# vribeiro1/artspeech

Measured on AMD Instinct MI355X. Metric: articulator-frames/sec (fwd+bwd), higher is better.
Workload: dtype f32

## Files before the change

artspeech_amd/_lib.py:

```python
import ctypes as C
import os

import torch

_HERE = os.path.dirname(os.path.abspath(__file__))
LIB_PATH = os.path.join(_HERE, "libartspeech_hip.so")

c_f32p = C.c_void_p


class Dims(C.Structure):
    _fields_ = [("vocab", C.c_int32), ("n_art", C.c_int32), ("embed", C.c_int32), ("hidden", C.c_int32),
                ("n_samp", C.c_int32), ("simple", C.c_int32)]


class Layout(C.Structure):
    _fields_ = [("embedding", C.c_int64),
                ("w_ih", C.c_int64 * 2), ("b_ih", C.c_int64 * 2), ("w_hh", C.c_int64 * 2), ("b_hh", C.c_int64 * 2),
                ("lin_w", C.c_int64), ("lin_b", C.c_int64),
                ("ln1_g", C.c_int64), ("ln1_b", C.c_int64), ("w1", C.c_int64), ("b1", C.c_int64),
                ("ln2_g", C.c_int64), ("ln2_b", C.c_int64), ("w2", C.c_int64), ("b2", C.c_int64),
                ("ln3_g", C.c_int64), ("ln3_b", C.c_int64), ("w3", C.c_int64), ("b3", C.c_int64),
                ("total", C.c_int64)]

# ... 22 lines not shown

class MultiMlp(C.Structure):
    _fields_ = [("groups", C.c_int32), ("rows", C.c_int32), ("layers", C.c_int32), ("h1", C.c_int32), ("h2", C.c_int32),
                ("k_max", C.c_int32), ("n_max", C.c_int32), ("latent", C.c_int32),
                ("dims", C.c_void_p), ("params", C.c_void_p), ("in_mode", C.c_int32), ("in_scale", C.c_float),
                ("x", C.c_void_p), ("x_r", C.c_int64), ("x_g", C.c_int64), ("in_idx", C.c_void_p),
                ("out_mode", C.c_int32), ("act", C.c_int32), ("y", C.c_void_p), ("y_r", C.c_int64), ("y_g", C.c_int64),
                ("out_idx", C.c_void_p), ("own_ptr", C.c_void_p), ("own", C.c_void_p), ("win", C.c_void_p),
                ("ws", C.c_void_p), ("ws_floats", C.c_int64), ("dy", C.c_void_p), ("dx", C.c_void_p), ("dparams", C.c_void_p)]


class Pca(C.Structure):
    _fields_ = [("groups", C.c_int32), ("features", C.c_int32), ("k_max", C.c_int32), ("batch", C.c_int32),
                ("k", C.c_void_p), ("x", C.c_void_p), ("rows", C.c_int64), ("x_r", C.c_int64), ("x_g", C.c_int64),
                ("order", C.c_void_p), ("n_seen", C.c_int64), ("state", C.c_void_p),
                ("components", C.c_void_p), ("singular_values", C.c_void_p), ("explained_variance", C.c_void_p),
                ("explained_variance_ratio", C.c_void_p), ("noise_variance", C.c_void_p),
                ("ws", C.c_void_p), ("ws_floats", C.c_int64)]


class Stream(C.c_void_p):
    from_param = C.c_void_p.from_param


_P, _S, _I32, _I64, _F, _D = C.c_void_p, Stream, C.c_int32, C.c_int64, C.c_float, C.c_double
_DIMS, _LAY = C.POINTER(Dims), C.POINTER(Layout)

PROTOTYPES = {
    "as_version": (C.c_char_p, []),
    "as_arch": (C.c_char_p, []),
    "as_last_error": (C.c_char_p, []),
    "as_artspeech_layout": (_I32, [_DIMS, _LAY]),
    "as_artspeech_workspace_floats": (_I64, [_DIMS, _I32, _I32]),
    "as_artspeech_fwd": (_I32, [_DIMS, _P, _P, _I64, _P, _I32, _I32, _P, _P, _I32, C.POINTER(Opts), _S]),
    "as_artspeech_bwd": (_I32, [_DIMS, _P, _P, _I64, _P, _I32, _I32, _P, _P, _P, _P, C.POINTER(Opts), _S]),
    "as_artspeech_dw2": (_I32, [_DIMS, _P, _I32, _I32, _P, _P, _S]),
    "as_gru_bidir_fwd": (_I32, [_P, _P, _I64, _P, _P, _P, _I32, _I32, _I32, _P, _P, _S]),
    "as_gru_bidir_bwd": (_I32, [_P, _P, _P, _P, _P, _I32, _I32, _I32, _P, _P, _S]),
    "as_gemm_f32": (_I32, [C.POINTER(Gemm), _S]),
    "as_linear_planes_floats": (_I64, [_I32, _I32]),
    "as_linear_fwd": (_I32, [_P, _I64, _P, _I64, _P, _P, _I64, _I32, _I32, _I32, _I32, _P, _S]),
    "as_layernorm_fwd_blockres": (_I32, [_P, _P, _P, _P, _I32, _I64, _I32, _I32, _S]),
    "as_head_workspace_floats": (_I64, [_DIMS, _I64]),
    "as_head_fwd": (_I32, [_DIMS, _LAY, _P, _P, _I64, _P, _P, _I32, _S]),
    "as_head_bwd": (_I32, [_DIMS, _LAY, _P, _P, _P, _I64, _P, _P, _P, _S]),
    "as_euclid_fwd": (_I32, [_P, _P, _I64, _I32, _I32, _P, _S]),
    "as_euclid_bwd": (_I32, [_P, _P, _P, _I64, _I32, _I32, _P, _S]),
    "as_euclid_masked_partials": (_I32, []),
    "as_euclid_masked_fwd_bwd": (_I32, [_P, _P, _I64, _P, _I32, _I32, _I32, _I32, _F, _P, _P, _P, _S]),
    "as_euclid_masked_fwd_bwd_presigmoid": (_I32, [_P, _P, _I64, _P, _I32, _I32, _I32, _I32, _F, _P, _P, _P, _S]),
    "as_p2cp_fwd": (_I32, [_P, _I64, _I64, _I64, _I32, _P, _I64, _I64, _I64, _I32, _I64, _P, _S]),
    "as_p2cp_bwd": (_I32, [_P, _I64, _I64, _I64, _I32, _P, _I64, _I64, _I64, _I32, _I64, _P, _P, _I64, _I64, _I64, _P, _I64, _I64, _I64,
                           _S]),
    "as_p2cp_masked_partials": (_I32, []),
    "as_p2cp_masked_fwd_bwd": (_I32, [_P, _P, _I64, _P, _I32, _I32, _I32, _I32, _F, _P, _P, _P, _S]),
    "as_p2cp_utterance_mean": (_I32, [_P, _P, _I32, _I32, _I32, _F, _P, _S]),
    "as_pearson_fwd": (_I32, [_P, _I64, _I64, _P, _I64, _I64, _I32, _I32, _I32, _I32, _F, _P, _P, _S]),
    "as_tract_variables_fwd": (_I32, [_P, _I64, _I32, _I32, _P, _I32, _P, _P, _P, _P, _S]),
    "as_area_function_fwd": (_I32, [_P, _P, _I64, _I64, _I64, _I64, _I32, _D, _D, _P, _P, _S]),
    "as_evenly_spaced_fx": (_I32, [_P, _P, _I64, _I32, _I32, _P, _S]),
    "as_adam_step": (_I32, [_P, _P, _P, _P, _I64, _F, _F, _F, _F, _F, _I64, _F, _S]),
    "as_dropout_fwd": (_I32, [_P, _P, _I64, _F, C.c_uint64, _S]),
    "as_layernorm_fwd": (_I32, [_P, _P, _P, _P, _P, _P, _P, _I64, _I32, _I64, _S]),
    "as_fold_ln": (_I32, [_P, _P, _P, _P, _P, _P, _I32, _I32, _I32, _S]),
    "as_attn_softmax": (_I32, [_P, _I64, _I32, _I32, _I32, _I32, _F, _P, _P, _S]),
    "as_embed_posenc": (_I32, [_P, _I64, _P, _P, _P, _I64, _I32, _I32, _S]),
    "as_attn_softmax_bwd": (_I32, [_P, _P, _I64, _I32, _I32, _F, _S]),
    "as_attention_supported": (_I32, [_I32, _I32, _I32, _I32]),
    "as_attention_fwd": (_I32, [_P, _P, _P, _P, _P, _P, _P, _P, _I32, _I32, _I32, _I32, _I32, _I32, _F, _S]),
    "as_attention_fwd_causal": (_I32, [_P, _P, _P, _P, _P, _P, _P, _P, _I32, _I32, _I32, _I32, _I32, _I32, _F, _S]),
    "as_attention_bwd_ds": (_I32, [_P, _P, _P, _P, _P, _I32, _I32, _I32, _I32, _I32, _I32, _F, _S]),
    "as_attention_bwd_ds_causal": (_I32, [_P, _P, _P, _P, _P, _I32, _I32, _I32, _I32, _I32, _I32, _F, _S]),
    "as_attn_softmax_bwd_t": (_I32, [_P, _P, _P, _P, _P, _I32, _I32, _I32, _I32, _I32, _I32, _F, _S]),
    "as_group_reduce": (_I32, [_P, _P, _I32, _I32, _I64, _P, _S]),
    "as_layernorm_bwd": (_I32, [_P, _P, _P, _P, _P, _I64, _I32, _S]),
    "as_unfold_ln": (_I32, [_P, _P, _P, _P, _P, _P, _P, _P, _I32, _I32, _I32, _S]),
    "as_relu_bwd": (_I32, [_P, _P, _P, _I64, _S]),
    "as_add": (_I32, [_P, _P, _P, _I64, _S]),
    "as_row_scale": (_I32, [_P, _P, _P, _I64, _I32, _S]),
    "as_copy_f32": (_I32, [_P, _P, _I64, _S]),
    "as_set_overlap": (None, [_I32]),
    "as_set_matrix_arith": (None, [_I32]),
    "as_get_matrix_arith": (_I32, []),
    "as_conv3x3_stem": (_I32, [_P, _I64, _I64, _I64, _I64, _P, _P, _P, _P, _I32, _I32, _I32, _I32, _S]),
    "as_conv3x3_c32": (_I32, [_P, _P, _P, _P, _P, _I32, _I32, _I32, _S]),
    "as_ln_feat_gelu": (_I32, [_P, _P, _P, _P, _I64, _I32, _I32, _S]),
    "as_gelu": (_I32, [_P, _P, _I64, _S]),
    "as_lstm_bidir_fwd": (_I32, [_P, _P, _I64, _P, _P, _P, _I32, _I32, _I32, _P, _P, _S]),
    "as_lstm_bidir_bwd": (_I32, [_P, _P, _P, _P, _I32, _I32, _I32, _P, _S]),
    "as_gru_unidir_fwd": (_I32, [_P, _P, _P, _P, _I32, _I32, _I32, _P, _S]),
    "as_gru_unidir_fwd_gates": (_I32, [_P, _P, _P, _P, _I32, _I32, _I32, _P, _P, _S]),
    "as_gru_unidir_bwd": (_I32, [_P, _P, _P, _P, _P, _I32, _I32, _I32, _P, _P, _S]),
    "as_ln_feat_gelu_bwd": (_I32, [_P, _P, _P, _P, _P, _P, _I64, _I32, _I32, _S]),
    "as_conv3x3_stem_bwd": (_I32, [_P, _P, _P, _I64, _I64, _I64, _I64, _I32, _I32, _I32, _I32, _S]),
    "as_gelu_bwd": (_I32, [_P, _P, _P, _P, _I64, _I32, _S]),
    "as_conv3x3_c32_wgrad": (_I32, [_P, _P, _P, _P, _I32, _I32, _I32, _P, _I64, _S]),
    "as_conv3x3_stem_wgrad": (_I32, [_P, _I64, _I64, _I64, _I64, _P, _P, _P, _I32, _I32, _I32, _I32, _P, _I64, _S]),
    "as_ln_feat_gelu_param_grad": (_I32, [_P, _P, _P, _P, _I64, _I32, _I32, _P, _P, _P, _I64, _S]),
    "as_layernorm_param_grad": (_I32, [_P, _P, _I64, _I32, _P, _P, _P, _I64, _S]),
    "as_ctc_workspace_floats": (_I64, [_I32, _I32, _I32]),
    "as_ctc_loss": (_I32, [_P, _I64, _I64, _I32, _I32, _I32, _I32, _P, _I64, _P, _P, _I32, _I32, _I32, _P, _I64, _P, _S]),
    "as_ctc_grad": (_I32, [_P, _I64, _I64, _I32, _I32, _I32, _I32, _P, _I64, _P, _P, _I32, _I32, _P, _I64, _P, _P, _I32, _P, _I64,
                           _I64, _S]),
    "as_decode_top1": (_I32, [_P, _I64, _I64, _I32, _I32, _I32, _P, _I32, _P, _P, _P, _S]),
    "as_edit_distance": (_I32, [_P, _I32, _P, _P, _I32, _P, _I32, _P, _I32, _P, _S]),
    "as_align_workspace_bytes": (_I64, [_I32, _I32, _I32]),
    "as_align_counts": (_I32, [_P, _I32, _P, _P, _I32, _P, _I32, _P, _I32, _I32, _P, _P, _P, _I64, _S]),
    "as_confusion_counts": (_I32, [_P, _I32, _P, _I32, _P, _I32, _P, _I32, _I32, _P, _S]),
    "as_intersect_semipolar_grid":(_I32, [_P, _P, _I64, _I32, _I32, _I32, _P, _P, _P, _S]),
    "as_artspeech_wait_head_grads": (_I32, [_P, _P]),
    "as_gather_pad_rows": (_I32, [_P, _P, _P, _I32, _I32, _I64, _I32, _D, _P, _S]),
    "as_lin_debug_stamps": (None, [_P, _I64]),
    "as_gru_debug_stamps": (None, [_P]),
    "as_multi_mlp_supported": (_I32, [_I32, _I32, _I32, _I32, _I32]),
    "as_multi_mlp_param_floats": (_I64, [_I32, _I32, _I32, _I32, _I32]),
    "as_multi_mlp_workspace_floats": (_I64, [C.POINTER(MultiMlp), _I32]),
    "as_multi_mlp_fwd": (_I32, [C.POINTER(MultiMlp), _S]),
    "as_multi_mlp_bwd": (_I32, [C.POINTER(MultiMlp), _S]),
    "as_pca_supported": (_I32, [_I32, _I32]),
    "as_pca_workspace_floats": (_I64, [C.POINTER(Pca)]),
    "as_pca_fit": (_I32, [C.POINTER(Pca), _S]),
    "as_token_runs_workspace_ints": (_I64, [_I64]),
    "as_token_runs": (_I32, [_P, _P, _P, _I32, _I64, _P, _P, _P, _P, _S]),
    "as_mean_contour_fit": (_I32, [_P, _P, _P, _P, _I32, _I32, _P, _P, _P, _S]),
    "as_mean_contour_fwd": (_I32, [_P, _P, _P, _P, _I32, _I32, _I32, _I32, _P, _P, _S]),
    "as_mean_contour_weighted_fwd": (_I32, [_P, _P, _P, _P, _P, _P, _I32, _I32, _I32, _I32, _P, _P, _S]),
    "as_pc_shapes_eval": (_I32, [_P, _P, _P, _P, _P, _I32, _P, _I32, _I64, _I32, _I32, _F, _P, _P, _P, _S]),
    "as_pc_eval_accumulate": (_I32, [_P, _I32, _P, _P, _I32, _P, _I64, _P, _I32, _S]),
    "as_segment_corr": (_I32, [_P, _P, _I64, _I32, _D, _P, _I32, _P, _P, _S]),
    "as_masked_mse_partials": (_I32, []),
    "as_masked_mse_fwd_bwd": (_I32, [_P, _P, _I64, _I64, _P, _I32, _P, _F, _P, _P, _P, _S]),
    "as_prepare_contours": (_I32, [_P, _P, _P, _I64, _I32, _I32, _F, _F, _F, _F, _P, _P, _I32, _P, _P, _P, _S]),
    "as_column_mean_std": (_I32, [_P, _I64, _I32, _P, _P, _P, _I64, _S]),
    "as_profile_enable": (None, [_I32]),
    "as_profile_reset": (None, []),
    "as_profile_report": (_I32, [C.c_char_p, _I32]),
}

COLUMN_STATS_PART_ROWS = 512

STATUS_WITHOUT_STREAM = ("as_artspeech_layout", "as_artspeech_wait_head_grads")

_lib = None
_bound = {}
_slabs = {}


def lib():
    global _lib
    if _lib is None:
        if not os.path.exists(LIB_PATH):
            raise RuntimeError(
                f"{LIB_PATH} is missing: build it with `python -m artspeech_amd.build` "
                "(hipcc --offload-arch=gfx950). artspeech_amd has no CPU fallback.")
        handle = C.CDLL(LIB_PATH, mode=C.RTLD_GLOBAL)
        for name, (res, args) in PROTOTYPES.items():
            fn = getattr(handle, name)
            fn.restype, fn.argtypes = res, args
            takes_stream = bool(args) and args[-1] is Stream
            _bound[name] = (fn, takes_stream, takes_stream or name in STATUS_WITHOUT_STREAM)
        _lib = handle
    return _lib


def check(rc, what=""):
    if rc != 0:
# ... 77 lines not shown
```

artspeech_amd/csrc/lin_f32.hip:

```cpp
#include <cstdlib>

#include <type_traits>

#include "gemm_internal.h"
#include "split_arith.h"

namespace {

constexpr int BN = 256, BK = 16, NT = 512, NBUF = 3;
enum { EPI_PLAIN = 0, EPI_LNF = 1, EPI_LNB = 2 };

struct LinK {
    const float* A; long lda, a_batch;
    const float* B; long ldb, b_batch;
    const uint16_t* Bp; long bp_plane, bp_batch; int bp_rows;
    int kchunk; long c_split;
    float* C; long ldc, c_batch;
    const float* bias; long bias_batch;
    int M, N, K, ka_valid, batch, act;
    int n_big, big_per_batch, big_per_batch_rows, small_per_batch;
    unsigned long long* dbg; long dbg_max;
    float eps;
    float* rstd;
    unsigned long long* bits;
    const float* xhat; long ldx, x_batch;
    const float* rstd_in;
    const unsigned long long* bits_in;
};

struct Tile { int bz, m0, tm; };
template <bool UNIFORM, typename K>
__device__ __forceinline__ Tile tile_of(const K& g) {
    const int tile = blockIdx.x;
    Tile t;
    if (tile < g.n_big) {
        t.bz = tile / g.big_per_batch;
        t.m0 = (tile - t.bz * g.big_per_batch) * 64;
        t.tm = 2;
    } else {
        const int j = tile - g.n_big;
        t.bz = j / g.small_per_batch;
        t.m0 = g.big_per_batch_rows + (j - t.bz * g.small_per_batch) * 32;
        t.tm = 1;
    }
    if (UNIFORM) {
        t.bz = __builtin_amdgcn_readfirstlane(t.bz);
        t.m0 = __builtin_amdgcn_readfirstlane(t.m0);
    }
    return t;
}

struct Stamps {
    unsigned long long* dbg;
    bool on;
    __device__ __forceinline__ Stamps(const LinK& g, int tid) : dbg(g.dbg), on(g.dbg != nullptr && tid == 0 && blockIdx.x < g.dbg_max) {}
    __device__ __forceinline__ unsigned long long* slot(int i) const { return on ? dbg + 8L * blockIdx.x + i : nullptr; }
    __device__ __forceinline__ void begin() const {
        if (!on) return;
        unsigned long long* d = slot(0);
        d[0] = __builtin_amdgcn_s_memtime();
        d[4] = __builtin_amdgcn_s_memrealtime();
        d[6] = 0;
        d[5] = __builtin_amdgcn_s_getreg((4 - 1) << 11 | 0 << 6 | 4) | ((unsigned long long)__builtin_amdgcn_s_getreg((32 - 1) << 11 | 0 << 6 | 20) << 32);
    }
    __device__ __forceinline__ void mark(int i) const {
        if (on) *slot(i) = __builtin_amdgcn_s_memtime();
    }
    __device__ __forceinline__ void end() const {
        if (!on) return;
        asm volatile("s_waitcnt vmcnt(0)" ::: "memory");
        *slot(3) = __builtin_amdgcn_s_memtime();
        *slot(6) = __builtin_amdgcn_s_memrealtime();
    }
};

template <int TM>
__device__ __forceinline__ void store_rows(const f32x16* acc, float* c0, long ld, float bj, int act, int m0, int M, int tm_eff, int lh) {
#pragma unroll
    for (int i = 0; i < TM; ++i)
#pragma unroll
        for (int r = 0; r < 16; ++r) {
            const int row = m0 + i * 32 + (r & 3) + 8 * (r >> 2) + 4 * lh;
            if (i < tm_eff && row < M) {
                float v = acc[i][r] + bj;
                if (act == 1) v = as_relu(v);
                else if (act == 2) v = as_sigmoid(v);
                c0[(long)row * ld] = v;
            }
        }
}

template <int TM, int EPI, int NWC>
__device__ __forceinline__ void lin_ln_rows(const LinK& g, f32x16 (&acc)[TM], float* smem, int bz, int m0, int tm_eff, int groups, int wave,
                                            int lane, float bj) {
    const int l31 = lane & 31, lh = lane >> 5;
    const int wave_u = __builtin_amdgcn_readfirstlane(wave);
    const int wn = wave_u % NWC, wm = wave_u / NWC;
    const int col = wn * 32 + l31;
    const int rr = lane >> 4, jj = lane & 15;
    constexpr float inv_d = 1.0f / BN;
    const int srow = 4 * wave_u + rr;
    const int trow_base = (srow >> 5) * 64 + (srow & 31);
    const bool stages = wm < groups, normalises = 4 * wave_u < 32 * groups;
// ... 283 lines not shown
    a_load(aq[0], 0);
    a_load(aq[1], 1);
    b_load(bq[0], 0);
    b_load(bq[1], 1);
    a_store(aq[0], 0);
    as_lds_barrier();
    if (stamp1) *stamp1 = __builtin_amdgcn_s_memtime();
    auto tile = [&](auto Uc, int kt) {
        constexpr int U = decltype(Uc)::value;
        const unsigned char* img = a_rd + (kt & 1) * S6_BUF;
        a_load(aq[(U + 2) % 3], kt + 2);
#pragma unroll
        for (int s = 0; s < 2; ++s) {
            b_load(bq[(2 * U + s + 2) % 3], 2 * kt + s + 2);
            __builtin_amdgcn_sched_barrier(0);
            bf16x8 fa[TME][3];
#pragma unroll
            for (int p = 0; p < 3; ++p)
#pragma unroll
                for (int i = 0; i < TME; ++i)
                    fa[i][p] = *reinterpret_cast<const bf16x8*>(img + p * S6_PLANE + i * 32 * 64 + (((2 * s + lh_rd) ^ sw) * 16));
            const u32x4(&bs)[3] = bq[(2 * U + s) % 3];
            bf16x8 fb[3];
#pragma unroll
            for (int p = 0; p < 3; ++p) fb[p] = __builtin_bit_cast(bf16x8, bs[p]);
            constexpr int PA[6] = {0, 0, 0, 1, 1, 2}, PB[6] = {0, 1, 2, 0, 1, 0};
#pragma unroll
            for (int o = 0; o < 6; ++o)
#pragma unroll
                for (int i = 0; i < TME; ++i)
                    acc[i] = __builtin_amdgcn_mfma_f32_32x32x16_bf16(fa[i][PA[o]], fb[PB[o]], acc[i], 0, 0, 0);
            __builtin_amdgcn_sched_barrier(0);
            if (late == (s == 0)) a_store(aq[(U + 1) % 3], (kt & 1) ^ 1);
        }
        as_lds_barrier();
    };
    int kt = 0;
    for (; kt + 3 <= nk; kt += 3) {
        tile(IC<0>{}, kt);
        tile(IC<1>{}, kt + 1);
        tile(IC<2>{}, kt + 2);
    }
    {
        int ln = lane;
        asm volatile("" : "+v"(ln));
        lh_rd = ln >> 5;
        sw = ((ln & 31) >> 2) & 3;
        a_rd = sm + (ln & 31) * 64;
    }
    if (kt < nk) tile(IC<0>{}, kt);
    if (kt + 1 < nk) tile(IC<1>{}, kt + 1);
}

template <int NW, typename K>
__device__ __forceinline__ void s6_tile(const K& g, const Tile& t, f32x16 (&acc)[2], unsigned char* sm, int k0, int klen, int kav, int tid,
                                        unsigned long long* stamp1 = nullptr) {
    const int lane = tid & 63, wave = tid >> 6;
#pragma unroll
    for (int i = 0; i < 2; ++i)
#pragma unroll
        for (int r = 0; r < 16; ++r) acc[i][r] = 0.f;
    const long bp_step = (long)g.bp_rows * 16;
    const uint16_t* bp = g.Bp + (long)t.bz * g.bp_batch + (k0 / 16) * bp_step;
    const unsigned b_lane = (unsigned)((wave * 32 + (lane & 31)) * 16 + (lane >> 5) * 8) * 2u;
    const float* A = g.A + (long)t.bz * g.a_batch + (long)t.m0 * g.lda + k0;
    const bool late = __builtin_amdgcn_readfirstlane(wave) >= NW / 2;
    if (t.tm == 2) s6_main_loop<NW, 2>(acc, sm, A, g.lda, g.M - t.m0, klen, kav, bp, b_lane, g.bp_plane, bp_step, tid, lane, late, stamp1);
    else s6_main_loop<NW, 1>(acc, sm, A, g.lda, g.M - t.m0, klen, kav, bp, b_lane, g.bp_plane, bp_step, tid, lane, late, stamp1);
}

template <int EPI>
__global__ __launch_bounds__(NT, 4) void lin_s6_kernel(LinK g) {
    constexpr int EPIT = 32 * BN;
    static_assert(EPIT * 4 >= 2 * S6_BUF, "the epilogue's staging area holds both plane images");
    __shared__ __attribute__((aligned(16))) float smem[EPIT];
    const Tile t = tile_of<true>(g);
    const int tid = threadIdx.x, lane = tid & 63, wave = tid >> 6;
    const Stamps stamps(g, tid);
    stamps.begin();
    f32x16 acc[2];
    s6_tile<8>(g, t, acc, reinterpret_cast<unsigned char*>(smem), 0, g.K, g.ka_valid, tid, stamps.slot(1));
    stamps.mark(2);
    lin_epilogue<2, EPI>(g, acc, smem, t.bz, t.m0, t.tm, wave, lane);
    stamps.end();
}

template <int NW, int WPS>
__global__ __launch_bounds__(NW * 64, WPS) void lin_s6_plain_kernel(LinK g) {
    __shared__ __attribute__((aligned(16))) unsigned char sm[2 * S6_BUF];
    const Tile t = tile_of<true>(g);
    const int tid = threadIdx.x, lane = tid & 63, wave = tid >> 6;
    const int ks = blockIdx.y, k0 = ks * g.kchunk;
    const int klen = min(g.kchunk, g.K - k0);
    f32x16 acc[2];
    s6_tile<NW>(g, t, acc, sm, k0, klen, max(0, min(klen, g.ka_valid - k0)), tid);
    const int col = wave * 32 + (lane & 31);
    if (col >= g.N) return;
    const bool whole = gridDim.y == 1;
    const float bj = (whole && g.bias) ? g.bias[(long)t.bz * g.bias_batch + col] : 0.f;
    store_rows<2>(acc, g.C + (long)ks * g.c_split + (long)t.bz * g.c_batch + col, g.ldc, bj, whole ? g.act : 0, t.m0, g.M, t.tm, lane >> 5);
}

constexpr int ON = 128;

struct LinOutK {
    const float* A; long lda, a_batch;
    const float* B; long ldb, b_batch; int b_rows;
    const float* bias; long bias_batch;
    float* out; long ldo, o_batch;
    int M, N, K, batch;
    int n_big, big_per_batch, big_per_batch_rows, small_per_batch;
    const float* tgt; long tgt_T; const int* lengths; int T; float scale;
    float* dout; float* partial;
    const uint16_t* Bp; long bp_plane, bp_batch; int bp_rows;
    float* loss; int* counter;
};

__device__ __forceinline__ void criterion_tail(const LinOutK& g, int tile, float sum, int tid, float* red) {
    if (g.counter == nullptr) {
        if (tid == 0) g.partial[tile] = sum;
        return;
    }
    __shared__ int s_last;
    if (tid == 0) {
        __hip_atomic_store(&g.partial[tile], sum, __ATOMIC_RELAXED, __HIP_MEMORY_SCOPE_AGENT);
        asm volatile("s_waitcnt vmcnt(0)" ::: "memory");
        const int last = atomicAdd(g.counter, 1) == (int)gridDim.x - 1;
        if (last) __hip_atomic_store(g.counter, 0, __ATOMIC_RELAXED, __HIP_MEMORY_SCOPE_AGENT);
        s_last = last;
    }
    __syncthreads();
    if (!s_last) return;
    float s = 0.f;
    if (tid < 256)
        for (int i = tid; i < (int)gridDim.x; i += 256) s += __hip_atomic_load(&g.partial[i], __ATOMIC_RELAXED, __HIP_MEMORY_SCOPE_AGENT);
    s = as_wave_sum(s);
    __syncthreads();
    if ((tid & 63) == 0 && tid < 256) red[tid >> 6] = s;
    __syncthreads();
    if (tid == 0) g.loss[0] = ((red[0] + red[1]) + (red[2] + red[3])) * g.scale;
}

static_assert(ON / 2 <= 64, "criterion_rows: a lane owns one point of a frame");
template <int NW>
__device__ __forceinline__ void criterion_rows(const LinOutK& g, const float* tile, const Tile& t, int tid) {
    constexpr int FPW = 64 / NW;
    static_assert(NW == 4 || NW == 8, "the workgroup sum below");
    const int lane = tid & 63, wave = tid >> 6;
    const int wave_u = __builtin_amdgcn_readfirstlane(wave);
    const int bz = t.bz, m0 = t.m0, rows = 32 * t.tm;
    const int Np = g.N >> 1;
    float part = 0.f;
    float tx[FPW], ty[FPW];
    bool in[FPW], valid[FPW];
    const int nl = min(lane, Np - 1);
#pragma unroll
    for (int k = 0; k < FPW; ++k) {
        const int r = wave_u + NW * k;
        const int frame = m0 + r;
        in[k] = r < rows && frame < g.M;
        const int fc = in[k] ? frame : m0;
        const int b = fc / g.T, t_ = fc - b * g.T;
        valid[k] = in[k] && t_ < g.lengths[b];
        const float* tg = g.tgt + (((long)b * g.tgt_T + t_) * g.batch + bz) * g.N;
        tx[k] = tg[nl];
        ty[k] = tg[Np + nl];
// ... 77 lines not shown
        if (active) {
#pragma unroll
            for (int cc = 0; cc < BK / 8; ++cc) {
                const int slot = ((2 * cc + lh) ^ swz) * 4;
                const float4 av = *reinterpret_cast<const float4*>(a_s + slot);
                const float4 bv = *reinterpret_cast<const float4*>(b_s + slot);
                acc = __builtin_amdgcn_mfma_f32_32x32x2f32(av.x, bv.x, acc, 0, 0, 0);
                acc = __builtin_amdgcn_mfma_f32_32x32x2f32(av.y, bv.y, acc, 0, 0, 0);
                acc = __builtin_amdgcn_mfma_f32_32x32x2f32(av.z, bv.z, acc, 0, 0, 0);
                acc = __builtin_amdgcn_mfma_f32_32x32x2f32(av.w, bv.w, acc, 0, 0, 0);
            }
        }
        if (kt + 2 < nk) asm volatile("s_waitcnt vmcnt(2)" ::: "memory");
        else asm volatile("s_waitcnt vmcnt(0)" ::: "memory");
        as_wait_lds();
        __builtin_amdgcn_s_barrier();
    }
    const int col = wn * 32 + l31;
    const float bj = (g.bias && col < g.N) ? g.bias[(long)bz * g.bias_batch + col] : 0.f;
    if (g.tgt == nullptr) {
        if (active && col < g.N) store_rows<1>(&acc, g.out + (long)bz * g.o_batch + col, g.ldo, bj, 2, m0 + wm * 32, g.M, 1, lh);
        return;
    }
    if (active) {
#pragma unroll
        for (int r = 0; r < 16; ++r) smem[(wm * 32 + (r & 3) + 8 * (r >> 2) + 4 * lh) * ON + col] = as_sigmoid(acc[r] + bj);
    }
    as_lds_barrier();
    criterion_rows<8>(g, smem, t, tid);
}

constexpr int LOUT_WPS = 3;
__global__ __launch_bounds__(256, LOUT_WPS) void lin_out_s6_kernel(LinOutK g) {
    __shared__ __attribute__((aligned(16))) float smem[64 * ON];
    static_assert(64 * ON * 4 >= 2 * S6_BUF, "the epilogue's tile holds both plane images");
    const Tile t = tile_of<true>(g);
    const int tid = threadIdx.x, lane = tid & 63, wave = tid >> 6;
    const int l31 = lane & 31, lh = lane >> 5;
    f32x16 acc[2];
    s6_tile<4>(g, t, acc, reinterpret_cast<unsigned char*>(smem), 0, g.K, g.K, tid);
    const int col = wave * 32 + l31;
    const float bj = (g.bias && col < g.N) ? g.bias[(long)t.bz * g.bias_batch + col] : 0.f;
    if (g.tgt == nullptr) {
        if (col < g.N) store_rows<2>(acc, g.out + (long)t.bz * g.o_batch + col, g.ldo, bj, 2, t.m0, g.M, t.tm, lh);
        return;
    }
#pragma unroll
    for (int i = 0; i < 2; ++i)
#pragma unroll
        for (int r = 0; r < 16; ++r)
            if (i < t.tm) smem[(i * 32 + (r & 3) + 8 * (r >> 2) + 4 * lh) * ON + col] = as_sigmoid(acc[i][r] + bj);
    as_lds_barrier();
    criterion_rows<4>(g, smem, t, tid);
}

template <typename K>
long tile_list(K& k, int x) {
    const int rest = k.M - x * 64;
    k.big_per_batch = x > 0 ? x : 1;
    k.big_per_batch_rows = x * 64;
    k.n_big = x * k.batch;
    k.small_per_batch = as_cdiv(rest, 32);
    const long total = (long)k.n_big + (long)k.small_per_batch * k.batch;
    if (k.small_per_batch == 0) k.small_per_batch = 1;
    return total;
}

int whole_round_tiles(int M, int batch, int slots, bool short_64) {
    const long units = (long)as_cdiv(M, 64) * batch;
    const long rounds = units / slots;
    if (rounds == 0 && short_64) return M / 64;
    const long x = rounds * slots / batch;
    return x > M / 64 ? M / 64 : (int)x;
}

template <typename K, typename L>
bool take_planes(K& k, const L* a, int min_rows) {
    if (!a->Bp || as_matrix_arith() != AS_ARITH_BF16X6 || a->K % S6_BK || a->bp_rows < min_rows || !as_aligned16(a->Bp) ||
        a->bp_plane % 8 || a->bp_batch % 8 || a->lda >= (1L << 23)) return false;
    k.Bp = a->Bp; k.bp_plane = a->bp_plane; k.bp_batch = a->bp_batch; k.bp_rows = a->bp_rows;
    return true;
}

unsigned long long* g_dbg = nullptr;
long g_dbg_max = 0;

LinK lin_args(const as_lin* a) {
    LinK k{};
    k.A = a->A; k.lda = a->lda; k.a_batch = a->a_batch;
    k.B = a->B; k.ldb = a->ldb; k.b_batch = a->b_batch;
    k.C = a->C; k.ldc = a->ldc; k.c_batch = a->c_batch;
    k.bias = a->bias; k.bias_batch = a->bias_batch;
    k.M = a->M; k.N = a->N; k.K = a->K; k.ka_valid = a->ka_valid > 0 ? a->ka_valid : a->K; k.batch = a->batch; k.act = a->act;
    k.eps = 1e-5f;
    k.dbg = g_dbg; k.dbg_max = g_dbg_max;
    k.rstd = a->rstd; k.bits = a->bits;
    k.xhat = a->xhat; k.ldx = a->ldx; k.x_batch = a->x_batch; k.rstd_in = a->rstd_in; k.bits_in = a->bits_in;
    return k;
}

template <bool B_KC, int EPI>
int launch(const LinK& k, hipStream_t st) {
    LinK kk = k;
    const long total = tile_list(kk, whole_round_tiles(k.M, k.batch, 512, false));
    if (kk.Bp) hipLaunchKernelGGL((lin_s6_kernel<EPI>), dim3((unsigned)total), dim3(NT), 0, st, kk);
    else hipLaunchKernelGGL((lin_f32_kernel<64, B_KC, EPI>), dim3((unsigned)total), dim3(NT), 0, st, kk);
    AS_LAUNCH_CHECK(kk.Bp ? "as_lin_s6" : "as_lin_f32");
    return 0;
}

}

extern "C" void as_lin_debug_stamps(uint64_t* buf, int64_t max_workgroups) {
    g_dbg = (unsigned long long*)buf;
    g_dbg_max = buf ? max_workgroups : 0;
}

int as_lin_try(const as_lin* a, hipStream_t st) {
    if (a->K % BK || a->K < BK || a->N > BN || a->N < 4 || a->M < 1 || a->batch < 1) return 0;
    if (!as_aligned16(a->A) || !as_aligned16(a->B) || a->lda % 4 || a->ldb % 4 || a->a_batch % 4 || a->b_batch % 4) return 0;
    if (!a->b_kc && a->N % 4) return 0;
    if (a->epi != EPI_PLAIN && (a->N != BN || !a->C)) return 0;
    if (a->epi == EPI_PLAIN && a->N <= BN / 2) return 0;
    if ((long)as_cdiv(a->M, 64) * a->batch > (1L << 30)) return 0;
    LinK k = lin_args(a);
    if (k.ka_valid % 4) return 0;
    take_planes(k, a, BN);
    if (a->epi == EPI_LNF) {
        if (!a->rstd || !a->bits || !a->b_kc) return 0;
        return launch<true, EPI_LNF>(k, st) == 0 ? 1 : -1;
    }
    if (a->epi == EPI_LNB) {
        if (!a->xhat || !a->rstd_in || !a->bits_in || a->b_kc) return 0;
        return launch<false, EPI_LNB>(k, st) == 0 ? 1 : -1;
    }
    if (a->b_kc) return launch<true, EPI_PLAIN>(k, st) == 0 ? 1 : -1;
    return launch<false, EPI_PLAIN>(k, st) == 0 ? 1 : -1;
}

int as_lin_plain_s6(const as_lin* a, int ksplit, long c_split, hipStream_t st, int waves_per_simd) {
    const int nw = a->N <= 128 ? 4 : 8;
    LinK k = lin_args(a);
    if (!take_planes(k, a, nw * 32)) return 0;
    if (a->epi != EPI_PLAIN || a->K < S6_BK || a->N > BN || a->N < 1 || a->M < 1 || a->batch < 1 || !a->C) return 0;
    if (!as_aligned16(a->A) || a->lda % 4 || a->a_batch % 4) return 0;
    if (ksplit < 1) ksplit = 1;
    if (ksplit > 1 && (a->bias || a->act)) return 0;
    if (k.ka_valid % 4) return 0;
    k.kchunk = (int)as_round_up(as_cdiv(a->K, ksplit), S6_BK);
    ksplit = as_cdiv(a->K, k.kchunk);
    k.c_split = c_split;
    const bool rows64 = (long)as_cdiv(a->M, 64) * a->batch * ksplit >= 384;
    const long total = tile_list(k, rows64 ? a->M / 64 : 0);
    if (total > (1L << 30) || ksplit > 65535) return 0;
    if (nw == 4 && waves_per_simd == 2) hipLaunchKernelGGL((lin_s6_plain_kernel<4, 2>), dim3((unsigned)total, ksplit), dim3(256), 0, st, k);
    else if (nw == 4) hipLaunchKernelGGL((lin_s6_plain_kernel<4, 4>), dim3((unsigned)total, ksplit), dim3(256), 0, st, k);
    else hipLaunchKernelGGL((lin_s6_plain_kernel<8, 4>), dim3((unsigned)total, ksplit), dim3(512), 0, st, k);
    AS_LAUNCH_CHECK("as_lin_plain_s6");
    return 1;
}

int as_lin_out_try(const as_lin_out* a, int* n_partials, hipStream_t st) {
    if (a->K % BK || a->K < BK || a->N > ON || a->N < 4 || a->N % 2 || a->M < 1 || a->batch < 1) return 0;
    if (!as_aligned16(a->A) || !as_aligned16(a->B) || a->lda % 4 || a->ldb % 4 || a->a_batch % 4 || a->b_batch % 4) return 0;
    if (a->b_rows < a->N) return 0;
    LinOutK k{};
    k.A = a->A; k.lda = a->lda; k.a_batch = a->a_batch;
    k.B = a->B; k.ldb = a->ldb; k.b_batch = a->b_batch; k.b_rows = a->b_rows;
    k.bias = a->bias; k.bias_batch = a->bias_batch;
    k.out = a->out; k.ldo = a->ldo; k.o_batch = a->o_batch;
    k.M = a->M; k.N = a->N; k.K = a->K; k.batch = a->batch;
    k.tgt = a->tgt; k.tgt_T = a->tgt_T; k.lengths = a->lengths; k.T = a->T; k.scale = a->scale; k.dout = a->dout; k.partial = a->partial;
    if (k.tgt && (!k.lengths || !k.dout || !k.partial || k.T < 1 || k.ldo != (long)k.batch * k.N || k.o_batch != k.N)) return 0;
    const long total = tile_list(k, whole_round_tiles(k.M, k.batch, 1024, true));
    if (k.tgt && total > a->partial_capacity) return 0;
    if (k.tgt && a->loss) {
        k.counter = as_arrival_counter(st);
        k.loss = k.counter ? a->loss : nullptr;
    }
    if (n_partials) *n_partials = k.counter ? 0 : (int)total;
    if (take_planes(k, a, ON)) hipLaunchKernelGGL(lin_out_s6_kernel, dim3((unsigned)total), dim3(256), 0, st, k);
    else hipLaunchKernelGGL(lin_out_kernel, dim3((unsigned)total), dim3(NT), 0, st, k);
    AS_LAUNCH_CHECK(k.Bp ? "as_lin_out_s6" : "as_lin_out");
    return 1;
}

namespace {
inline bool linear_blocks(int N, int* bn, int* nb) {
    if (N <= 256) { *bn = N <= 128 ? 128 : 256; *nb = 1; return true; }
    if (N % 256 == 0) { *bn = 256; *nb = N / 256; return true; }
    return false;
}
}

extern "C" int64_t as_linear_planes_floats(int32_t N, int32_t K) {
    int bn, nb;
    if (N < 1 || K < 1 || !linear_blocks(N, &bn, &nb)) return 0;
    return as_round_up(as_planes_floats(nb, bn, (int)as_round_up(K, 32)), 64);
}
// ... 29 lines not shown
```

include/artspeech_hip.h:

```cpp
#ifndef ARTSPEECH_HIP_H
#define ARTSPEECH_HIP_H

#include <stdint.h>

#ifdef __cplusplus
extern "C" {
#endif

#define AS_ERR_BAD_ARG (-1)
#define AS_ERR_UNSUPPORTED (-2)
#define AS_ERR_WORKSPACE (-3)

#define AS_HEAD_HIDDEN 256

const char* as_version(void);
const char* as_arch(void);
const char* as_last_error(void);

typedef struct as_dims {
    int32_t vocab;
    int32_t n_art;
    int32_t embed;
    int32_t hidden;
    int32_t n_samp;
    int32_t simple;
} as_dims;

typedef struct as_layout {
    int64_t embedding;
    int64_t w_ih[2], b_ih[2];
    int64_t w_hh[2], b_hh[2];
    int64_t lin_w, lin_b;
    int64_t ln1_g, ln1_b;
    int64_t w1, b1;
    int64_t ln2_g, ln2_b;
    int64_t w2, b2;
    int64_t ln3_g, ln3_b;
    int64_t w3, b3;
    int64_t total;
} as_layout;

int as_artspeech_layout(const as_dims* dims, as_layout* out);

int64_t as_artspeech_workspace_floats(const as_dims* dims, int32_t B, int32_t T);

typedef struct as_opts {
    float gru_dropout;
    uint64_t dropout_seed;
    int32_t dout_presigmoid;
    int32_t defer_dw2;
    void* fold_wait_event;
    const float* loss_targets; int64_t loss_tgt_T; float loss_scale; float* loss_out; float* loss_dout;
} as_opts;

int as_artspeech_fwd(const as_dims* dims, const float* params, const int64_t* tokens, int64_t tok_stride,
                     const int32_t* lengths, int32_t B, int32_t T, float* out, float* ws, int32_t train,
                     const as_opts* opts, void* stream);

int as_artspeech_bwd(const as_dims* dims, const float* params, const int64_t* tokens, int64_t tok_stride,
                     const int32_t* lengths, int32_t B, int32_t T, const float* out, const float* dout,
                     float* grads, float* ws, const as_opts* opts, void* stream);

int as_artspeech_dw2(const as_dims* dims, const float* params, int32_t B, int32_t T, float* grads, float* ws, void* stream);

void as_set_overlap(int32_t on);

int as_copy_f32(const float* src, float* dst, int64_t n, void* stream);

void as_set_matrix_arith(int32_t mode);
int32_t as_get_matrix_arith(void);

int as_artspeech_wait_head_grads(void* compute_stream, void* waiting_stream);


int as_gru_bidir_fwd(const float* gi, const int64_t* tokens, int64_t tok_stride, const float* w_hh,
                     const float* b_hh, const int32_t* lengths, int32_t B, int32_t T, int32_t H, float* y,
                     float* gates, void* stream);

int as_gru_bidir_bwd(const float* dy, const float* y, const float* gates, const float* w_hh,
                     const int32_t* lengths, int32_t B, int32_t T, int32_t H, float* dgi, float* dgh,
                     void* stream);

int as_lstm_bidir_fwd(const float* gi, const int64_t* tokens, int64_t tok_stride, const float* w_hh, const float* b_hh,
                      const int32_t* lengths, int32_t B, int32_t T, int32_t H, float* y, float* gates, void* stream);
int as_lstm_bidir_bwd(const float* dy, const float* gates, const float* w_hh, const int32_t* lengths, int32_t B, int32_t T,
                      int32_t H, float* dg, void* stream);

typedef struct as_gemm {
    const float* A; const float* B; float* C; const float* bias;
    int32_t M, N, K;
    int64_t a_i, a_k, b_j, b_k, ldc;
    int32_t batch; int64_t a_batch, b_batch, c_batch, bias_batch;
    int32_t act, accumulate;
    int32_t b_kshift, b_kT;
    float* splitk_ws; int64_t splitk_ws_floats;
    float* colsum; int64_t colsum_batch;
    const int64_t* a_off; const int64_t* b_off; const int64_t* c_off; const int64_t* bias_off;
    int32_t precision;
    int32_t b_kshift_batch;
    int32_t cu_budget;
    const float* res; int64_t res_ld, res_batch; const int64_t* res_off;
    const uint32_t* mask_bits; int64_t mask_batch;
    uint32_t* relu_bits; int64_t relu_bits_batch;
    int32_t k_seg; const int64_t* a_seg_off; const int64_t* b_seg_off;
    int32_t k_tri;
} as_gemm;
int as_gemm_f32(const as_gemm* g, void* stream);

int64_t as_linear_planes_floats(int32_t N, int32_t K);
int as_linear_fwd(const float* A, int64_t lda, const float* W, int64_t ldw, const float* bias, float* out, int64_t ldo,
                  int32_t M, int32_t N, int32_t K, int32_t act, float* planes_ws, void* stream);

int64_t as_head_workspace_floats(const as_dims* dims, int64_t rows);
int as_head_fwd(const as_dims* dims, const as_layout* lay, const float* params, const float* x, int64_t rows,
                float* out, float* ws, int32_t train, void* stream);
int as_head_bwd(const as_dims* dims, const as_layout* lay, const float* params, const float* out,
                const float* dout, int64_t rows, float* dx, float* grads, float* ws, void* stream);

int as_euclid_fwd(const float* out, const float* tgt, int64_t frames, int32_t A, int32_t N, float* dist,
                  void* stream);
int as_euclid_bwd(const float* out, const float* tgt, const float* ddist, int64_t frames, int32_t A, int32_t N,
                  float* dout, void* stream);

int32_t as_euclid_masked_partials(void);
int as_euclid_masked_fwd_bwd(const float* out, const float* tgt, int64_t tgt_T, const int32_t* lengths, int32_t B,
                             int32_t T, int32_t A, int32_t N, float scale, float* loss, float* dout,
                             float* partial, void* stream);
int as_euclid_masked_fwd_bwd_presigmoid(const float* out, const float* tgt, int64_t tgt_T, const int32_t* lengths, int32_t B,
                             int32_t T, int32_t A, int32_t N, float scale, float* loss, float* dout,
                             float* partial, void* stream);

int as_p2cp_fwd(const float* u, int64_t u_tile, int64_t u_pt, int64_t u_xy, int32_t n_u, const float* v,
                int64_t v_tile, int64_t v_pt, int64_t v_xy, int32_t n_v, int64_t tiles, float* out, void* stream);

int as_p2cp_bwd(const float* u, int64_t u_tile, int64_t u_pt, int64_t u_xy, int32_t n_u, const float* v, int64_t v_tile,
                int64_t v_pt, int64_t v_xy, int32_t n_v, int64_t tiles, const float* dout, float* du, int64_t du_tile,
                int64_t du_pt, int64_t du_xy, float* dv, int64_t dv_tile, int64_t dv_pt, int64_t dv_xy, void* stream);

int32_t as_p2cp_masked_partials(void);
int as_p2cp_masked_fwd_bwd(const float* out, const float* tgt, int64_t tgt_T, const int32_t* lengths, int32_t B, int32_t T,
                           int32_t A, int32_t N, float scale, float* loss, float* dout, float* partial, void* stream);

int as_p2cp_utterance_mean(const float* p2cp, const int32_t* lengths, int32_t B, int32_t T, int32_t A, float to_mm,
                           float* result, void* stream);

int as_pearson_fwd(const float* out, int64_t out_b, int64_t out_t, const float* tgt, int64_t tgt_b, int64_t tgt_t,
                   int32_t B, int32_t T, int32_t A, int32_t N, float eps, float* x_corr, float* y_corr, void* stream);

int as_tract_variables_fwd(const float* contours, int64_t frames, int32_t A, int32_t N, const int32_t* spec,
                           int32_t n_tv, float* values, float* poc1, float* poc2, int32_t* idx, void* stream);

int as_area_function_fwd(const double* internal_wall, const double* external_wall, int64_t frame_stride,
                         int64_t pt_stride, int64_t xy_stride, int64_t frames, int32_t n_pts, double alpha,
// ... 192 lines not shown
```

Baseline: 6.532 million.

## Add short-K resident-A split-bf16 kernels for layernorm-fused head linears

Adds specialized kernels for the head's layernorm-fused linear layers when K is at most 128. The whole A tile is loaded once, split into three bf16 planes and kept resident in LDS. For the forward LNF case with a shared (unbatched) A, one workgroup loops over several heads and reuses that resident A image instead of reloading and re-splitting it per head. The B planes are prefetched through a small register ring. The change adds a runtime toggle (on by default), more dynamic LDS use and extra code paths, and the larger LDS footprint may lower occupancy.

New measurement: 6.633 million, median of 6. +1.5%, better.

```diff
diff --git a/artspeech_amd/_lib.py b/artspeech_amd/_lib.py
--- a/artspeech_amd/_lib.py
+++ b/artspeech_amd/_lib.py
@@ -128,6 +128,7 @@
     "as_set_overlap": (None, [_I32]),
     "as_set_matrix_arith": (None, [_I32]),
     "as_get_matrix_arith": (_I32, []),
+    "as_set_head_short_k": (None, [_I32]),
     "as_conv3x3_stem": (_I32, [_P, _I64, _I64, _I64, _I64, _P, _P, _P, _P, _I32, _I32, _I32, _I32, _S]),
     "as_conv3x3_c32": (_I32, [_P, _P, _P, _P, _P, _I32, _I32, _I32, _S]),
     "as_ln_feat_gelu": (_I32, [_P, _P, _P, _P, _I64, _I32, _I32, _S]),
diff --git a/artspeech_amd/csrc/lin_f32.hip b/artspeech_amd/csrc/lin_f32.hip
--- a/artspeech_amd/csrc/lin_f32.hip
+++ b/artspeech_amd/csrc/lin_f32.hip
@@ -1,7 +1,9 @@
 #include <cstdlib>
 
+#include <atomic>
 #include <type_traits>
 
+#include "as_launch.h"
 #include "gemm_internal.h"
 #include "split_arith.h"
 
@@ -19,6 +21,7 @@
     const float* bias; long bias_batch;
     int M, N, K, ka_valid, batch, act;
     int n_big, big_per_batch, big_per_batch_rows, small_per_batch;
+    int groups;
     unsigned long long* dbg; long dbg_max;
     float eps;
     float* rstd;
@@ -468,6 +471,172 @@
     s6_tile<8>(g, t, acc, reinterpret_cast<unsigned char*>(smem), 0, g.K, g.ka_valid, tid, stamps.slot(1));
     stamps.mark(2);
     lin_epilogue<2, EPI>(g, acc, smem, t.bz, t.m0, t.tm, wave, lane);
+    stamps.end();
+}
+
+constexpr int S6R_MAXK = 128, S6R_MAXT = S6R_MAXK / S6_BK;
+
+__device__ __forceinline__ void s6r_image_load(f32x4 (&aq)[S6R_MAXT], const float* __restrict__ A, long lda, int rows_valid, int nk, int ka_valid,
+                                               int tid) {
+    const int a_chunk = tid & 7, row = tid >> 3;
+    const unsigned a_off = (unsigned)(min(row, rows_valid - 1) * (int)lda + a_chunk * 4) * 4u;
+    const gptr Au = as_uniform_ptr(A);
+#pragma unroll
+    for (int q = 0; q < S6R_MAXT; ++q) {
+        const int kt = min(q, nk - 1);
+        const unsigned ko = kt * S6_BK + a_chunk * 4 + 4 <= ka_valid ? (unsigned)(kt * S6_BK) * 4u : 0u - (unsigned)a_chunk * 16u;
+        aq[q] = *reinterpret_cast<gptr_f4>(Au + (a_off + ko));
+    }
+}
+__device__ __forceinline__ void s6r_image_store(const f32x4 (&aq)[S6R_MAXT], unsigned char* sm, int nk, int tid) {
+    const int a_chunk = tid & 7, row = tid >> 3;
+    const int a_wr = row * 64 + (((a_chunk >> 1) ^ ((row >> 2) & 3)) * 16) + (a_chunk & 1) * 8;
+#pragma unroll
+    for (int q = 0; q < S6R_MAXT; ++q) {
+        unsigned h0, m0, l0, h1, m1, l1;
+        split_pair(aq[q].x, aq[q].y, h0, m0, l0);
+        split_pair(aq[q].z, aq[q].w, h1, m1, l1);
+        unsigned char* d = sm + min(q, nk - 1) * S6_BUF + a_wr;
+        *reinterpret_cast<uint2*>(d) = make_uint2(h0, h1);
+        *reinterpret_cast<uint2*>(d + S6_PLANE) = make_uint2(m0, m1);
+        *reinterpret_cast<uint2*>(d + 2 * S6_PLANE) = make_uint2(l0, l1);
+    }
+}
+
+struct S6B { const uint16_t* bp; long bp_plane, bp_step; unsigned b_lane; int nj; };
+template <typename K>
+__device__ __forceinline__ S6B s6_b_of(const K& g, int bz, int nk, int tid) {
+    const int lane = tid & 63, wave = tid >> 6;
+    S6B b;
+    b.bp_step = (long)g.bp_rows * 16;
+    b.bp = g.Bp + (long)bz * g.bp_batch;
+    b.bp_plane = g.bp_plane;
+    b.b_lane = (unsigned)((wave * 32 + (lane & 31)) * 16 + (lane >> 5) * 8) * 2u;
+    b.nj = 2 * nk;
+    return b;
+}
+__device__ __forceinline__ void s6_b_load(u32x4 (&dst)[3], const S6B& b, int j) {
+    j = min(j, b.nj - 1);
+#pragma unroll
+    for (int p = 0; p < 3; ++p) dst[p] = *reinterpret_cast<gptr_u4>(as_uniform_ptr(b.bp + p * b.bp_plane + j * b.bp_step) + b.b_lane);
+}
+
+template <int TME>
+__device__ __forceinline__ void s6_resident_loop(f32x16 (&acc)[2], const unsigned char* sm, int nk, const S6B& b, u32x4 (&bq)[3][3], int lane) {
+    const int l31 = lane & 31;
+    int sw = (l31 >> 2) & 3;
+    const unsigned char* a_rd = sm + l31 * 64;
+    int lh_rd = lane >> 5;
+    auto tile = [&](auto Uc, int kt) {
+        constexpr int U = decltype(Uc)::value;
+        const unsigned char* img = a_rd + kt * S6_BUF;
+#pragma unroll
+        for (int s = 0; s < 2; ++s) {
+            s6_b_load(bq[(2 * U + s + 2) % 3], b, 2 * kt + s + 2);
+            __builtin_amdgcn_sched_barrier(0);
+            bf16x8 fa[TME][3];
+#pragma unroll
+            for (int p = 0; p < 3; ++p)
+#pragma unroll
+                for (int i = 0; i < TME; ++i)
+                    fa[i][p] = *reinterpret_cast<const bf16x8*>(img + p * S6_PLANE + i * 32 * 64 + (((2 * s + lh_rd) ^ sw) * 16));
+            const u32x4(&bs)[3] = bq[(2 * U + s) % 3];
+            bf16x8 fb[3];
+#pragma unroll
+            for (int p = 0; p < 3; ++p) fb[p] = __builtin_bit_cast(bf16x8, bs[p]);
+            constexpr int PA[6] = {0, 0, 0, 1, 1, 2}, PB[6] = {0, 1, 2, 0, 1, 0};
+#pragma unroll
+            for (int o = 0; o < 6; ++o)
+#pragma unroll
+                for (int i = 0; i < TME; ++i)
+                    acc[i] = __builtin_amdgcn_mfma_f32_32x32x16_bf16(fa[i][PA[o]], fb[PB[o]], acc[i], 0, 0, 0);
+            __builtin_amdgcn_sched_barrier(0);
+        }
+    };
+    int kt = 0;
+    if (nk >= 3) {
+        tile(IC<0>{}, 0);
+        tile(IC<1>{}, 1);
+        tile(IC<2>{}, 2);
+        kt = 3;
+    }
+    {
+        int ln = lane;
+        asm volatile("" : "+v"(ln));
+        lh_rd = ln >> 5;
+        sw = ((ln & 31) >> 2) & 3;
+        a_rd = sm + (ln & 31) * 64;
+    }
+    if (kt < nk) tile(IC<0>{}, kt);
+    if (kt + 1 < nk) tile(IC<1>{}, kt + 1);
+}
+__device__ __forceinline__ void s6_zero(f32x16 (&acc)[2]) {
+#pragma unroll
+    for (int i = 0; i < 2; ++i)
+#pragma unroll
+        for (int r = 0; r < 16; ++r) acc[i][r] = 0.f;
+}
+
+__global__ __launch_bounds__(NT, 4) void lin_s6_lnf_shared_kernel(LinK g) {
+    extern __shared__ __attribute__((aligned(16))) unsigned char dsm[];
+    const Tile t = tile_of<true>(g);
+    const int tid = threadIdx.x, lane = tid & 63, wave = tid >> 6;
+    const Stamps stamps(g, tid);
+    stamps.begin();
+    const int nk = g.K / S6_BK;
+    float* stage = reinterpret_cast<float*>(dsm + nk * S6_BUF);
+    const int h0 = t.bz * g.batch / g.groups, h1 = (t.bz + 1) * g.batch / g.groups;
+    f32x4 aq[S6R_MAXT];
+    u32x4 bq[3][3];
+    s6r_image_load(aq, g.A + (long)t.m0 * g.lda, g.lda, g.M - t.m0, nk, g.ka_valid, tid);
+    S6B b = s6_b_of(g, h0, nk, tid);
+    s6_b_load(bq[0], b, 0);
+    s6_b_load(bq[1], b, 1);
+    s6r_image_store(aq, dsm, nk, tid);
+    as_lds_barrier();
+    stamps.mark(1);
+    const int col = wave * 32 + (lane & 31);
+    for (int h = h0; h < h1; ++h) {
+        f32x16 acc[2];
+        s6_zero(acc);
+        if (t.tm == 2) s6_resident_loop<2>(acc, dsm, nk, b, bq, lane);
+        else s6_resident_loop<1>(acc, dsm, nk, b, bq, lane);
+        b = s6_b_of(g, min(h + 1, h1 - 1), nk, tid);
+        s6_b_load(bq[0], b, 0);
+        s6_b_load(bq[1], b, 1);
+        const float bj = g.bias ? g.bias[(long)h * g.bias_batch + col] : 0.f;
+        if (h > h0) as_lds_barrier();
+        lin_ln_rows<2, EPI_LNF, 8>(g, acc, stage, h, t.m0, t.tm, 1, wave, lane, bj);
+    }
+    stamps.mark(2);
+    stamps.end();
+}
+
+__global__ __launch_bounds__(NT, 4) void lin_s6_lnb_short_kernel(LinK g) {
+    constexpr int EPIT = 32 * BN;
+    __shared__ __attribute__((aligned(16))) unsigned char sm[S6R_MAXT * S6_BUF];
+    static_assert(S6R_MAXT * S6_BUF >= EPIT * 4, "the image's memory holds the epilogue's staging area");
+    const Tile t = tile_of<true>(g);
+    const int tid = threadIdx.x, lane = tid & 63, wave = tid >> 6;
+    const Stamps stamps(g, tid);
+    stamps.begin();
+    const int nk = g.K / S6_BK;
+    f32x4 aq[S6R_MAXT];
+    u32x4 bq[3][3];
+    s6r_image_load(aq, g.A + (long)t.bz * g.a_batch + (long)t.m0 * g.lda, g.lda, g.M - t.m0, nk, g.ka_valid, tid);
+    const S6B b = s6_b_of(g, t.bz, nk, tid);
+    s6_b_load(bq[0], b, 0);
+    s6_b_load(bq[1], b, 1);
+    s6r_image_store(aq, sm, nk, tid);
+    as_lds_barrier();
+    stamps.mark(1);
+    f32x16 acc[2];
+    s6_zero(acc);
+    if (t.tm == 2) s6_resident_loop<2>(acc, sm, nk, b, bq, lane);
+    else s6_resident_loop<1>(acc, sm, nk, b, bq, lane);
+    stamps.mark(2);
+    as_lds_barrier();
+    lin_ln_rows<2, EPI_LNB, 8>(g, acc, reinterpret_cast<float*>(sm), t.bz, t.m0, t.tm, 1, wave, lane, 0.f);
     stamps.end();
 }
 
@@ -711,6 +880,8 @@
     return true;
 }
 
+std::atomic<int> g_short_k{1};
+
 unsigned long long* g_dbg = nullptr;
 long g_dbg_max = 0;
 
@@ -728,8 +899,39 @@
     return k;
 }
 
+
+int launch_short_k(const LinK& k, int epi, hipStream_t st, bool* took) {
+    *took = false;
+    if (!g_short_k.load(std::memory_order_relaxed) || !k.Bp || k.K > S6R_MAXK) return 0;
+    LinK kk = k;
+    if (epi == EPI_LNB) {
+        const long total = tile_list(kk, whole_round_tiles(k.M, k.batch, 512, false));
+        hipLaunchKernelGGL(lin_s6_lnb_short_kernel, dim3((unsigned)total), dim3(NT), 0, st, kk);
+        AS_LAUNCH_CHECK("as_lin_s6_lnb_short");
+        *took = true;
+        return 0;
+    }
+    if (epi != EPI_LNF || k.a_batch != 0) return 0;
+    const int lds = (k.K / S6_BK) * S6_BUF + 32 * BN * 4;
+    if (lds > 64 * 1024 && as_allow_dynamic_lds(lin_s6_lnf_shared_kernel, lds) != hipSuccess) return 0;
+    const int row_tiles = as_cdiv(k.M, 64);
+    kk.groups = 512 / row_tiles < 1 ? 1 : 512 / row_tiles > k.batch ? k.batch : 512 / row_tiles;
+    kk.batch = kk.groups;
+    const long total = tile_list(kk, (long)row_tiles * kk.groups >= 384 ? k.M / 64 : 0);
+    kk.batch = k.batch;
+    hipLaunchKernelGGL(lin_s6_lnf_shared_kernel, dim3((unsigned)total), dim3(NT), lds, st, kk);
+    AS_LAUNCH_CHECK("as_lin_s6_lnf_shared");
+    *took = true;
+    return 0;
+}
+
 template <bool B_KC, int EPI>
 int launch(const LinK& k, hipStream_t st) {
+    if (EPI != EPI_PLAIN) {
+        bool took;
+        const int e = launch_short_k(k, EPI, st, &took);
+        if (e || took) return e;
+    }
     LinK kk = k;
     const long total = tile_list(kk, whole_round_tiles(k.M, k.batch, 512, false));
     if (kk.Bp) hipLaunchKernelGGL((lin_s6_kernel<EPI>), dim3((unsigned)total), dim3(NT), 0, st, kk);
@@ -744,6 +946,8 @@
     g_dbg = (unsigned long long*)buf;
     g_dbg_max = buf ? max_workgroups : 0;
 }
+
+extern "C" void as_set_head_short_k(int32_t on) { g_short_k.store(on ? 1 : 0, std::memory_order_relaxed); }
 
 int as_lin_try(const as_lin* a, hipStream_t st) {
     if (a->K % BK || a->K < BK || a->N > BN || a->N < 4 || a->M < 1 || a->batch < 1) return 0;
diff --git a/include/artspeech_hip.h b/include/artspeech_hip.h
--- a/include/artspeech_hip.h
+++ b/include/artspeech_hip.h
@@ -69,6 +69,8 @@
 
 void as_set_matrix_arith(int32_t mode);
 int32_t as_get_matrix_arith(void);
+
+void as_set_head_short_k(int32_t on);
 
 int as_artspeech_wait_head_grads(void* compute_stream, void* waiting_stream);
 
```
